# JuliaGraphics/Hikari.jl

Hardware: AMD Instinct MI355X
Metric: Mrays/s (higher is better)
Workload: dtype f32

## Files before the change

hikari.jl_amd/csrc/hk_kernels.hip:

```cpp
#include <hip/hip_runtime.h>
#include <type_traits>
#include <cstdlib>
#include <cstdio>

#include "hikari_mi355x.h"
#include "hk_device.h"
#include "hk_edit_host.h"
#include "hk_bvh_decide.h"

using namespace hkd;

namespace {

__device__ __forceinline__ int lane_id() { return (int)(threadIdx.x & 63); }

struct WaveQ {
    uint32_t* base;
    int count;
};
__device__ __forceinline__ int global_wave() {
    const int w = (int)(threadIdx.x >> 6), b = (int)blockIdx.x;
    if (blockDim.x == 1024 && (gridDim.x & 7) == 0) return ((((b >> 3) * 4 + (w >> 2)) * 8 + (b & 7)) << 2) + (w & 3);
    if (blockDim.x == 512 && (gridDim.x & 7) == 0) return ((((b >> 3) * 2 + (w >> 2)) * 8 + (b & 7)) << 2) + (w & 3);
    return b * (int)(blockDim.x >> 6) + w;
// ... 2197 lines not shown
                    if (descend) {
                        const int at = __popcll(dm & lt_mask);
                        pool[0][at] = e;
                        pool[1][at] = __float_as_uint(sp.x), pool[2][at] = __float_as_uint(sp.y), pool[3][at] = __float_as_uint(sp.z);
                        pool[4][at] = __float_as_uint(sn.x), pool[5][at] = __float_as_uint(sn.y), pool[6][at] = __float_as_uint(sn.z);
                        pool[7][at] = __float_as_uint(u_b);
                    }
                    pool_n = __popcll(dm);
                    __builtin_amdgcn_wave_barrier();
                }
            }
            const int avail = pool_n - pool_head;
            if (avail > 0) {
                const int rank = __popcll(free_m & lt_mask);
                if (!busy && rank < avail) {
                    const int at = pool_head + rank;
                    slot = pool[0][at];
                    p = mk3(__uint_as_float(pool[1][at]), __uint_as_float(pool[2][at]), __uint_as_float(pool[3][at]));
                    nn = mk3(__uint_as_float(pool[4][at]), __uint_as_float(pool[5][at]), __uint_as_float(pool[6][at]));
                    ub = __uint_as_float(pool[7][at]);
                    pmf = 1.0f - p_inf;
                    bits = root_bits, child = root_child;
                    lvl = 0;
                    busy = true;
                }
                const int free_n = __popcll(free_m);
                pool_head += free_n < avail ? free_n : avail;
            }
            if (__ballot(busy) == 0ull) {
                if (!more && pool_head == pool_n) break;
                continue;
            }
        }
        if (busy) {
            int res_light = -1;
            float res_pmf = 0.0f;
            if (lvl >= 64) {
                res_light = 0;
            } else {
                ++lvl;
                DLightNode n0, n1;
                if (NTOP > 0 && (int)child + 1 < n_top) {
                    n0 = lds_light_node<NTOP>(top, (int)child), n1 = lds_light_node<NTOP>(top, (int)child + 1);
                    asm volatile("" : "+v"(n0.bits));
                } else
                    n0 = load_light_node(sc.lnodes, (int)child), n1 = load_light_node(sc.lnodes, (int)child + 1);
                const float c0 = node_importance(n0, p, nn);
                const float c1 = node_importance(n1, p, nn);
                n_lnodes += 2;
                if (c0 == 0.0f && c1 == 0.0f) {
                    res_light = 0;
                } else {
                    const float p0 = c0 / (c0 + c1);
                    if (ub < p0) {
                        pmf *= p0;
                        ub = ub / p0;
                        bits = n0.bits, child = n0.child1_or_light;
                    } else {
                        pmf *= (1.0f - p0);
                        ub = (ub - p0) / (1.0f - p0);
                        bits = n1.bits, child = n1.child1_or_light;
                    }
                    if ((bits & 2u) && lvl < 64) {
                        res_light = (int)child;
                        res_pmf = pmf;
                    }
                }
            }
            if (res_light >= 0) {
                st.sel_light[slot] = make_uint2((uint32_t)res_light, __float_as_uint(res_pmf));
                busy = false;
            }
        }
    }
    stats += global_wave();
    wave_add(&stats->light_nodes, n_lnodes);
}

#ifndef HK_SHADE_WAVES_MATTE
#define HK_SHADE_WAVES_MATTE 4
#endif
#ifndef HK_SHADE_WAVES
#define HK_SHADE_WAVES 3
#endif
#ifndef HK_SHADE_WAVES_LEAN
#define HK_SHADE_WAVES_LEAN 5
#endif
#ifndef HK_SHADE_WAVES_LEAN_HASH
#define HK_SHADE_WAVES_LEAN_HASH 5
#endif
template <bool TWO_PLANES, bool SIMPLE, bool LEAN = false>
HKD void shade_emission(const DPathState& st, const DPathGen& g, bool ones, const DScene& sc, const DTables& T, uint32_t slot, unsigned& n_lnodes, int depth, size_t seg) {
    const float4 H = st.hit[slot];
    const float4 O = ld_ray_o(st, g, slot, depth, seg), D = g.ray_d[slot];
    const v3 ro = mk3(O.x, O.y, O.z), rd = mk3(D.x, D.y, D.z);
    const float t_hit = H.x;
    const int prim = __float_as_int(H.y);
    const DTriMeta meta = tri_meta(sc, prim);
    if (meta.arealight <= 0) return;
    const Surface sf = surface_at(sc, prim, H.z, H.w, ro, rd, t_hit);
    const v3 wo = -rd;
    uint2 pmeta;
    if constexpr (LEAN) {
        const uint32_t w = reinterpret_cast<const uint32_t*>(g.meta)[slot];
        pmeta = make_uint2((uint32_t)depth | (((w >> 30) & 1u) << 8), w & 0x3fffffffu);
    } else
        pmeta = ld_meta(st, g, slot, depth);
    const S4 lambda = ld_lambda(st, g, slot, pmeta.y);
    const DLight& light = sc.lights[meta.arealight - 1];
    S4 Le = arealight_Le<TWO_PLANES, SIMPLE>(sc, T, light, wo, sf.n, sf.uv, lambda);
    if (is_black(Le)) return;
    const S4 beta = ld_throughput(g.beta, slot, ones);
    const uint32_t fl = pmeta.x;
    const int pdepth = (int)(fl & 0xff);
    const bool specular_bounce = (fl >> 8) & 1u;
    S4 contribution = beta * Le;
    S4 fin;
    if constexpr (LEAN) {
        fin = contribution;
        if (!(pdepth == 0 || specular_bounce)) {
            const float r_l = ones ? 1.0f : D.w;
            float choice = bvh_pmf(sc, sf.pi, sf.n, (int)meta.arealight, n_lnodes);
            float ct = fabsf(dot(sf.n, normalize(rd)));
            float light_pdf = 0.0f;
            if (ct > 0.0f && sf.area > 0.0f) light_pdf = choice * ((t_hit * t_hit) / (ct * sf.area));
            const float a = 1.0f + r_l * light_pdf;
            const float den = (((a + a) + a) + a) / 4.0f;
            if (den > 1e-10f) fin = contribution / den;
        }
    } else {
        const S4 r_u = ld_ru(g, slot, ones, st.compact != 0), r_l = ld_rl(g, slot, ones, st.compact != 0);
        if (pdepth == 0 || specular_bounce)
            fin = contribution / average(r_u);
        else {
            float choice = bvh_pmf(sc, sf.pi, sf.n, (int)meta.arealight, n_lnodes);
            float ct = fabsf(dot(sf.n, normalize(rd)));
            float light_pdf = 0.0f;
            if (ct > 0.0f && sf.area > 0.0f) light_pdf = choice * ((t_hit * t_hit) / (ct * sf.area));
            S4 rl = r_l * light_pdf;
            float den = average(r_u + rl);
            fin = den > 1e-10f ? contribution / den : contribution / average(r_u);
        }
    }
    st4(&st.L[pmeta.y], ld4(&st.L[pmeta.y]) + fin);
}

template <int KIND>
struct ShadeWaves {
    static constexpr int value = (KIND == HK_MAT_COATED_DIFFUSE || KIND == HK_MAT_COATED_DIFFUSE_TRANSMISSION) ? 1 : (KIND == HK_MAT_MATTE ? HK_SHADE_WAVES_MATTE : HK_SHADE_WAVES);
};
#ifndef HK_SHADE_MIN_WAVES
#define HK_SHADE_MIN_WAVES 1
#endif
#define HK_SHADE_STASH 16
struct ShadeStage {
    uint32_t* entry;
    float4* hit;
    float4* ray_d;
    uint32_t* meta;
};
__device__ __forceinline__ void lds_fetch4(const uint32_t* src, uint32_t* lds_wave_base) {
    __builtin_amdgcn_global_load_lds((const __attribute__((address_space(1))) void*)src, (__attribute__((address_space(3))) void*)lds_wave_base, 4, 0, 0);
}
__device__ __forceinline__ void lds_fetch16(const float4* src, float4* lds_wave_base) {
    __builtin_amdgcn_global_load_lds((const __attribute__((address_space(1))) void*)src, (__attribute__((address_space(3))) void*)lds_wave_base, 16, 0, 0);
}
template <int KIND, bool SIMPLE, bool FT, bool PRE, bool LEAN = false>
__device__ __forceinline__ void shade_body(const DPathState& st, const DScene& sc, const DTables& T, const DFrame& fr, const DSobol& sob, int depth, int first_kind, DStats* stats, const SegTickets& src,
                                           uint32_t* __restrict__ elist,
                                           float* stash = nullptr,
                                           ShadeStage stage = ShadeStage{}) {
    static_assert(!LEAN || (KIND == HK_MAT_MATTE && HK_LAMBDA_BY_SLOT), "the lean body is Matte's");
    const int lane = lane_id();
    unsigned n_vertices = 0, n_lnodes = 0;
    unsigned nv_wave = 0;
    unsigned* const nl_stash = LEAN ? reinterpret_cast<unsigned*>(stash) + (HK_SHADE_STASH - 1) * 256 + threadIdx.x : nullptr;
    auto nl_flush = [&]() {
        if constexpr (LEAN) {
            if (n_lnodes) *nl_stash += n_lnodes;
            n_lnodes = 0;
        }
    };
    if constexpr (LEAN) *nl_stash = 0u;
    auto uni = [](int v) { return LEAN ? __builtin_amdgcn_readfirstlane(v) : v; };
    HK_FOR_EACH_SEGMENT_FROM(gw_v, st, src) {
    const int gw = uni(gw_v);
    const uint32_t* __restrict__ queue = st.mat_q + ((size_t)KIND * st.n_waves + gw) * st.wave_cap;
    const int n = uni(*count_ptr(st, depth, Q_MAT0 + KIND, gw));
    const DPathGen g = gen_at(st, depth), gn = st.gen[(depth + 1) & 1];
    const size_t seg = (size_t)gw * st.wave_cap;
    const bool ones = depth == 0 && fr.implicit_ones;
    WavePos q_shadow{0}, q_next{0};
    if (!first_kind) {
        q_shadow.count = uni(*count_ptr(st, depth, Q_SHADOW, gw));
        q_next.count = uni(*count_ptr(st, depth + 1, Q_RAY, gw));
    }
    int n_emit = 0;
    auto emit_pass = [&](int take) {
        __builtin_amdgcn_fence(__ATOMIC_SEQ_CST, "wavefront");
        if (lane < take) shade_emission<KIND == HK_MAT_MATTE, SIMPLE, LEAN>(st, g, ones, sc, T, elist[lane], n_lnodes, depth, seg);
        nl_flush();
        const int rest = n_emit - take;
        const uint32_t moved = lane < rest ? elist[64 + lane] : 0u;
        __builtin_amdgcn_fence(__ATOMIC_SEQ_CST, "wavefront");
        if (lane < rest) elist[lane] = moved;
        n_emit = rest;
    };
    const bool prescan = uni(st.shade_prescan) != 0;
    if (prescan) {
        for (int base = 0; base < n || n_emit > 0; base += 64) {
            if (base < n) {
                const int i = base + lane;
                const uint32_t cand = i < n ? queue[i] & ~HK_MATQ_EMISSIVE : 0u;
                const bool em = i < n && (st.mat_id[cand] & HK_MAT_EMISSIVE_BIT) != 0;
                const unsigned long long m = __ballot(em);
                if (em) elist[n_emit + __popcll(m & ((1ull << lane) - 1ull))] = cand;
                n_emit += __popcll(m);
                if (n_emit < 64 && base + 64 < n) continue;
            }
            emit_pass(n_emit < 64 ? n_emit : 64);
        }
    }
    const bool prefetch = LEAN && stage.entry != nullptr;
    const int wave0 = LEAN ? __builtin_amdgcn_readfirstlane((int)(threadIdx.x & ~63u)) : 0;
    if constexpr (LEAN) {
        if (prefetch && 64 + lane < n) lds_fetch4(&queue[64 + lane], stage.entry + 256 + wave0);
    }
    for (int base = 0; base < n; base += 64) {
        int i = base + lane;
        bool active = i < n;
        if constexpr (LEAN) {
            if (prefetch && i + 128 < n) lds_fetch4(&queue[i + 128], stage.entry + ((base >> 6) & 1) * 256 + wave0);
        }
        const bool staged = prefetch && base > 0;
        uint32_t slot = active ? queue[i] : 0u;
        {
            const bool em = !prescan && (slot & HK_MATQ_EMISSIVE) != 0u;
            slot &= ~HK_MATQ_EMISSIVE;
            const unsigned long long m = __ballot(em);
            if (m != 0ull) {
                if (em) elist[n_emit + __popcll(m & ((1ull << lane) - 1ull))] = slot;
                n_emit += __popcll(m);
                if (n_emit >= 64) emit_pass(64);
            }
        }
        bool push_shadow = false, push_ray = false;
        float4 H = make_float4(0, 0, 0, 0);
        Surface sf;
        v3 wo = mk3(0, 0, 1);
        DTriMeta meta{0u, 0u, 0u};
        S4 lambda = s4(0.0f), beta = s4(0.0f), r_u = s4(0.0f), kd_matte = s4(0.0f);
        uint32_t fl = 0, pslot = 0;
        int pdepth = 0, medium = -1;
        bool any_non_specular = false;
        SobolCtx sctx;
        using W = std::conditional_t<LEAN, float, S4>;
        auto stash_at = [&]() {
            int i = (int)threadIdx.x;
            asm volatile("" : "+v"(i));
            return stash + i;
        };
        const int base_dim = 6 + 7 * depth;
        float4 shO = make_float4(0, 0, 0, 0), shD = shO;
        S4 shLd = s4(0.0f);
        W shRu{}, shRl{};
        if constexpr (LEAN) nv_wave += (unsigned)(n - base < 64 ? n - base : 64);
        if (active) {
            if constexpr (!LEAN) ++n_vertices;
            float4 D;
            uint32_t meta_w = 0;
            if (LEAN && staged) {
                asm volatile("s_waitcnt vmcnt(0)" ::: "memory");
                const int t = (int)threadIdx.x;
                H = stage.hit[t], D = stage.ray_d[t], meta_w = stage.meta[t];
            } else {
                H = stream_ld(&st.hit[slot]);
                D = stream_ld(&g.ray_d[slot]);
                if constexpr (LEAN) meta_w = reinterpret_cast<const uint32_t*>(g.meta)[slot];
            }
            float4 O = ld_ray_o(st, g, slot, depth, seg);
            v3 ro = mk3(O.x, O.y, O.z), rd = mk3(D.x, D.y, D.z);
            float t_hit = H.x;
            int prim = __float_as_int(H.y);
            sf = surface_at(sc, prim, H.z, H.w, ro, rd, t_hit);
            wo = -rd;
            meta = tri_meta(sc, prim);
            if constexpr (LEAN) {
                pslot = meta_w & 0x3fffffffu;
                pdepth = depth;
                any_non_specular = (meta_w >> 31) != 0u;
            } else {
                const uint2 pmeta = ld_meta(st, g, slot, depth);
                fl = pmeta.x;
                pslot = pmeta.y;
                pdepth = (int)(fl & 0xff);
                any_non_specular = (fl >> 9) & 1u;
                medium = (int)(fl >> 16) - 1;
                r_u = ld_ru(g, slot, ones, st.compact != 0);
            }
            lambda = ld_lambda(st, g, slot, pslot);
            if (ones)
                beta = s4(1.0f);
            else {
                const float4 bv = stream_ld(&g.beta[slot]);
                beta = s4(bv.x, bv.y, bv.z, bv.w);
            }

            int pix, k;
            split_slot(fr, pslot, pix, k);
            sctx = sobol_ctx_slot(sob, T.sobol, fr.x0, fr.y0, fr.tiles_x, pix, k, fr.first_sample + k * fr.sample_stride);

            if (KIND == HK_MAT_MATTE) kd_matte = matte_kd<SIMPLE>(sc, T, sc.materials[st.mat_id[slot] & ~HK_MAT_EMISSIVE_BIT], TexCtx(sf.uv, meta.prim_index, H.z, H.w), lambda);
#ifdef HK_ABLATE
            {
                float sink = 0.0f;
                if (HK_ABLATE == 1) {
                    uint32_t ps2 = pslot;
                    int d2 = base_dim;
                    asm volatile("" : "+v"(ps2));
                    asm volatile("" : "+s"(d2));
                    int pix2, k2;
                    split_slot(fr, ps2, pix2, k2);
                    SobolCtx c2 = sobol_ctx_slot(sob, T.sobol, fr.x0, fr.y0, fr.tiles_x, pix2, k2, fr.first_sample + k2 * fr.sample_stride);
                    v2 a = sobol_2d(c2, d2 + 3), b = sobol_2d(c2, d2 + 6);
                    sink = sobol_1d(c2, d2 + 1) + a.x + a.y + b.x + b.y + sobol_1d(c2, d2 + 7);
                }
                if (HK_ABLATE == 2 && sc.n_lights > 0) {
                    float u2 = H.z, pmf2;
                    asm volatile("" : "+v"(u2));
                    unsigned dummy = 0;
                    sink = (float)bvh_sample_light(sc, sf.pi, sf.ns, u2, pmf2, dummy) + pmf2;
                }
                if (HK_ABLATE == 3 && sc.n_lights > 0) {
                    uint32_t li = pslot;
                    asm volatile("" : "+v"(li));
                    LightSample l2 = sample_light(sc, T, sc.lights[li % (uint32_t)sc.n_lights], sf.pi, lambda, mk2(H.z, H.w));
                    sink = l2.pdf + l2.Li.x + l2.Li.w + l2.wi.x + l2.p_light.z;
                }
                if (HK_ABLATE == 4) {
                    S4 l2 = lambda;
                    asm volatile("" : "+v"(l2.x), "+v"(l2.y), "+v"(l2.z), "+v"(l2.w));
                    S4 k2 = matte_kd(sc, T, sc.materials[st.mat_id[slot] & ~HK_MAT_EMISSIVE_BIT], TexCtx(sf.uv, meta.prim_index, H.z, H.w), l2);
                    sink = k2.x + k2.y + k2.z + k2.w;
                }
                if (HK_ABLATE == 5) {
                    float b2 = H.z;
                    asm volatile("" : "+v"(b2));
                    Surface s2 = surface_at(sc, prim, b2, H.w, ro, rd, t_hit);
                    sink = s2.pi.x + s2.n.y + s2.ns.z + s2.uv.x + s2.area;
                }
                if (HK_ABLATE == 6) {
                    v3 w2 = wo;
                    asm volatile("" : "+v"(w2.x), "+v"(w2.y), "+v"(w2.z));
                    float p2;
                    S4 f2 = eval_matte_kd(kd_matte, w2, sf.n, sf.ns, p2);
                    BSDFSample s2 = sample_matte_kd(sc, sc.materials[st.mat_id[slot] & ~HK_MAT_EMISSIVE_BIT], kd_matte, w2, sf.ns, TexCtx(sf.uv, meta.prim_index, H.z, H.w), mk2(H.z, H.w));
                    sink = f2.x + f2.w + p2 + s2.pdf + s2.wi.x + s2.f.y;
                }
                asm volatile("" : : "v"(sink));
            }
#endif

            if constexpr (LEAN) {
                float* sp = stash + threadIdx.x;
                sp[0 * 256] = sf.n.x, sp[1 * 256] = sf.n.y, sp[2 * 256] = sf.n.z;
                sp[3 * 256] = wo.x, sp[4 * 256] = wo.y, sp[5 * 256] = wo.z;
                sp[6 * 256] = kd_matte.x, sp[7 * 256] = kd_matte.y, sp[8 * 256] = kd_matte.z, sp[9 * 256] = kd_matte.w;
                sp[10 * 256] = beta.x, sp[11 * 256] = beta.y, sp[12 * 256] = beta.z, sp[13 * 256] = beta.w;
                sp[14 * 256] = __uint_as_float(meta_w);
                if (prefetch && i + 64 < n) {
                    asm volatile("s_waitcnt vmcnt(0)" ::: "memory");
                    const uint32_t ns = stage.entry[(((base >> 6) + 1) & 1) * 256 + (int)threadIdx.x] & ~HK_MATQ_EMISSIVE;
                    lds_fetch16(&st.hit[ns], stage.hit + wave0);
                    lds_fetch16(&g.ray_d[ns], stage.ray_d + wave0);
                    lds_fetch4(reinterpret_cast<const uint32_t*>(g.meta) + ns, stage.meta + wave0);
                }
            }
            if (sc.n_lights > 0) {
                const DMaterial& mat = sc.materials[st.mat_id[slot] & ~HK_MAT_EMISSIVE_BIT];
                float light_pmf;
                int light_idx;
                if constexpr (PRE) {
                    const uint2 pre = st.sel_light[slot];
                    light_idx = (int)pre.x;
                    light_pmf = __uint_as_float(pre.y);
                } else {
                    float light_select = sobol_1d<FT>(sctx, base_dim + 1);
                    light_idx = bvh_sample_light(sc, sf.pi, sf.ns, light_select, light_pmf, n_lnodes);
                }
                if (light_idx >= 1 && light_idx <= sc.n_lights && light_pmf > 0.0f) {
                    const DLight& sel = sc.lights[light_idx - 1];
                    v2 u_light = mk2(0.0f, 0.0f);
                    if (sel.kind >= HK_LIGHT_AMBIENT) u_light = sobol_2d<FT>(sctx, base_dim + 3);
                    LightSample ls = sample_light<KIND == HK_MAT_MATTE, SIMPLE>(sc, T, sel, sf.pi, lambda, u_light);
                    if (ls.pdf > 0.0f && !is_black(ls.Li)) {
                        float bsdf_pdf;
                        if constexpr (LEAN) {
                            const float* sp = stash_at();
                            wo = mk3(sp[3 * 256], sp[4 * 256], sp[5 * 256]);
                            kd_matte = s4(sp[6 * 256], sp[7 * 256], sp[8 * 256], sp[9 * 256]);
                            beta = s4(sp[10 * 256], sp[11 * 256], sp[12 * 256], sp[13 * 256]);
                        }
                        S4 f = KIND == HK_MAT_MATTE ? eval_matte_kd(kd_matte, wo, ls.wi, sf.ns, bsdf_pdf)
                                                    : eval_bsdf<KIND>(sc, T, mat, wo, ls.wi, sf.ns, TexCtx(sf.uv, meta.prim_index, H.z, H.w), lambda, bsdf_pdf);
                        if (!is_black(f)) {
                            float ct = fabsf(dot(ls.wi, sf.ns));
                            S4 Ld = beta * f * ls.Li * ct;
                            if (!is_black(Ld)) {
                                v3 off = 1e-4f * sf.ns;
                                v3 so = dot(ls.wi, sf.ns) > 0.0f ? sf.pi + off : sf.pi - off;
                                v3 tl = ls.p_light - so;
                                float tmax = sqrtf(dot(tl, tl)) - 1e-3f;
                                float nbp = ls.is_delta ? 0.0f : bsdf_pdf;
                                shO = make_float4(so.x, so.y, so.z, tmax);
                                shD = make_float4(ls.wi.x, ls.wi.y, ls.wi.z, __int_as_float(medium));
                                shLd = Ld;
                                if constexpr (LEAN) {
                                    shRu = nbp;
                                    shRl = ls.pdf * light_pmf;
                                } else {
                                    shRu = r_u * nbp;
                                    shRl = (r_u * ls.pdf) * light_pmf;
                                }
                                push_shadow = true;
                            }
                        }
                    }
                }
            }
        }
        nl_flush();
        {
            const size_t ps = seg + (size_t)wp_push(q_shadow, push_shadow);
            if constexpr (LEAN) {
                if (push_shadow) {
                    const float m = shRu + shRl;
                    shD.w = (((m + m) + m) + m) / 4.0f;
                    stream_st(&st.sh_o[ps], shO);
                    stream_st(&st.sh_d[ps], shD);
                    stream_st(&st.sh_Ld[ps], shLd);
                    stream_st(&st.sh_slot[ps], pslot);
                }
            } else if (push_shadow && st.sh_final) {
                const S4 mis = s4(shRu.x) * s4(1.0f) + s4(shRl.x) * s4(1.0f);
                shD.w = average(mis);
                stream_st(&st.sh_o[ps], shO);
                stream_st(&st.sh_d[ps], shD);
                stream_st(&st.sh_Ld[ps], shLd);
                stream_st(&st.sh_slot[ps], pslot);
            } else if (push_shadow) {
                stream_st(&st.sh_o[ps], shO);
                stream_st(&st.sh_d[ps], shD);
                stream_st(&st.sh_Ld[ps], shLd);
                if (st.compact) {
#if HK_NT
                    __builtin_nontemporal_store((hk_f2){shRu.x, shRl.x}, (hk_f2*)(reinterpret_cast<float2*>(st.sh_ru) + ps));
#else
                    reinterpret_cast<float2*>(st.sh_ru)[ps] = make_float2(shRu.x, shRl.x);
#endif
                } else
                    st_shadow_weights(st, ps, shRu, shRl);
                stream_st(&st.sh_slot[ps], pslot);
            }
        }
        float4 nO = make_float4(0, 0, 0, 0), nD = nO;
        S4 nb = s4(0.0f);
        W nrl{};
        uint32_t nflags = 0;
        if (active) {
            int new_depth = pdepth + 1;
            if (new_depth < fr.max_depth) {
                const DMaterial& mat = sc.materials[st.mat_id[slot] & ~HK_MAT_EMISSIVE_BIT];
                DMediumInterface mi{};
                if constexpr (LEAN) {
                    const float* sp = stash_at();
                    sf.n = mk3(sp[0 * 256], sp[1 * 256], sp[2 * 256]);
                    wo = mk3(sp[3 * 256], sp[4 * 256], sp[5 * 256]);
                    kd_matte = s4(sp[6 * 256], sp[7 * 256], sp[8 * 256], sp[9 * 256]);
                    beta = s4(sp[10 * 256], sp[11 * 256], sp[12 * 256], sp[13 * 256]);
                    const uint32_t meta_w = __float_as_uint(sp[14 * 256]);
                    pslot = meta_w & 0x3fffffffu;
                    any_non_specular = (meta_w >> 31) != 0u;
                    int pix, k;
                    split_slot(fr, pslot, pix, k);
                    sctx = sobol_ctx_slot(sob, T.sobol, fr.x0, fr.y0, fr.tiles_x, pix, k, fr.first_sample + k * fr.sample_stride);
                } else
                    mi = sc.mis[meta.mi];
                float uc = (KIND == HK_MAT_GLASS || KIND > HK_MAT_CONDUCTOR) && KIND != HK_MAT_FALLBACK ? sobol_1d<FT>(sctx, base_dim + 4) : 0.0f;
                v2 u = (KIND == HK_MAT_MIRROR || KIND == HK_MAT_GLASS || KIND == HK_MAT_THIN_DIELECTRIC) ? mk2(0.0f, 0.0f) : sobol_2d<FT>(sctx, base_dim + 6);
                bool regularize = fr.regularize && any_non_specular;
                BSDFSample s = KIND == HK_MAT_MATTE ? sample_matte_kd<SIMPLE>(sc, mat, kd_matte, wo, sf.ns, TexCtx(sf.uv, meta.prim_index, H.z, H.w), u)
                                                    : sample_bsdf<KIND>(sc, T, mat, wo, sf.ns, TexCtx(sf.uv, meta.prim_index, H.z, H.w), lambda, u, uc, regularize);
                if (s.pdf > 0.0f && !is_black(s.f)) {
                    float ct = fabsf(dot(s.wi, sf.ns));
                    nb = s.is_specular ? beta * s.f : beta * s.f * ct / s.pdf;
                    if constexpr (LEAN) nrl = s.is_specular ? 1.0f : 1.0f / s.pdf;
                    else nrl = s.is_specular ? r_u : r_u / s.pdf;
                    bool cont = true;
                    if (new_depth > 3) {
                        float rr = sobol_1d<FT>(sctx, base_dim + 7);
                        float q = maxf(0.05f, 1.0f - max_component(nb));
                        if (rr < q)
                            cont = false;
                        else
                            nb = nb * (1.0f / (1.0f - q));
                    }
                    if (cont) {
                        int new_medium = -1;
                        if constexpr (!LEAN) new_medium = (mi.inside != mi.outside) ? (dot(s.wi, sf.n) > 0.0f ? mi.outside : mi.inside) : medium;
                        v3 off = dot(s.wi, sf.n) > 0.0f ? sf.n : -sf.n;
                        v3 no = sf.pi + off * 0.0001f;
                        nO = make_float4(no.x, no.y, no.z, INF_F);
                        nD = make_float4(s.wi.x, s.wi.y, s.wi.z, 0.0f);
                        bool ans = any_non_specular || !s.is_specular;
                        nflags = (uint32_t)new_depth | ((s.is_specular ? 1u : 0u) << 8) | ((ans ? 1u : 0u) << 9) | ((uint32_t)(new_medium + 1) << 16);
                        push_ray = true;
                    }
                }
            }
        }
        {
            const size_t pn = seg + (size_t)wp_push(q_next, push_ray);
            if constexpr (LEAN) {
                if (push_ray) {
                    stream_st(&gn.ray_o[pn], nO);
                    nD.w = nrl;
                    stream_st(&gn.ray_d[pn], nD);
                    stream_st(&gn.beta[pn], nb);
                    stream_st(reinterpret_cast<uint32_t*>(gn.meta) + pn, pslot | (((nflags >> 8) & 1u) << 30) | (((nflags >> 9) & 1u) << 31));
                }
            } else if (push_ray) {
                stream_st(&gn.ray_o[pn], nO);
                if (st.compact) nD.w = nrl.x;
                stream_st(&gn.ray_d[pn], nD);
                stream_st(&gn.beta[pn], nb);
                st_ru_rl(gn, pn, r_u, nrl, st.compact != 0);
                st_lambda(gn, pn, lambda);
                st_meta(st, gn, pn, nflags, pslot);
            }
        }
    }
    if (n_emit > 0) emit_pass(n_emit);
    if (lane == 0) {
        *count_ptr(st, depth, Q_SHADOW, gw) = q_shadow.count;
        *count_ptr(st, depth + 1, Q_RAY, gw) = q_next.count;
    }
    }
    if constexpr (LEAN) {
        n_vertices = lane == 0 ? nv_wave : 0u;
        n_lnodes = *nl_stash;
    }
    stats += global_wave();
    wave_add(&stats->vertices, n_vertices);
    wave_add(&stats->light_nodes, n_lnodes);
}
template <int KIND, bool SIMPLE = false, bool FT = false, bool PRE = false, bool LEAN = false>
__global__ void __attribute__((amdgpu_flat_work_group_size(256, 256), amdgpu_waves_per_eu(LEAN ? (FT ? HK_SHADE_WAVES_LEAN : HK_SHADE_WAVES_LEAN_HASH) : ShadeWaves<KIND>::value))) k_shade(DPathState st, DScene sc, DTables T, DFrame fr, DSobol sob, int depth, int first_kind, DStats* stats) {
    __shared__ uint32_t emit_list[4 * 128];
    SegTickets src = seg_open(st, ticket_ptr(st, depth, TK_SHADE0 + KIND), st.dynamic_segments != 0, depth, Q_MAT0 + KIND);
    if constexpr (LEAN) {
        src.pos = __builtin_amdgcn_readfirstlane(src.pos), src.k0 = __builtin_amdgcn_readfirstlane(src.k0);
        __shared__ float stash[HK_SHADE_STASH * 256];
        __shared__ uint32_t stage_entry[2 * 256];
        __shared__ float4 stage_hit[256];
        __shared__ float4 stage_ray_d[256];
        __shared__ uint32_t stage_meta[256];
        ShadeStage stage{};
        if (st.shade_prefetch) stage.entry = stage_entry, stage.hit = stage_hit, stage.ray_d = stage_ray_d, stage.meta = stage_meta;
        shade_body<KIND, SIMPLE, FT, PRE, true>(st, sc, T, fr, sob, depth, first_kind, stats, src, emit_list + (threadIdx.x >> 6) * 128, stash, stage);
    } else
        shade_body<KIND, SIMPLE, FT, PRE>(st, sc, T, fr, sob, depth, first_kind, stats, src, emit_list + (threadIdx.x >> 6) * 128);
}

template <class W> HKD W wone();
template <> HKD float wone<float>() { return 1.0f; }
template <> HKD S4 wone<S4>() { return s4(1.0f); }
HKD S4 wide(S4 v) { return v; }
HKD S4 wide(float v) { return s4(v); }
HKD bool is_black(float v) { return v == 0.0f; }
template <bool COMPACT>
HKD void shadow_contribute(const DPathState& st, uint32_t rec, S4 T_ray, S4 tr_u, S4 tr_l) {
    if (is_black(T_ray)) return;
    S4 w_u, w_l;
    ld_shadow_weights<COMPACT>(st, rec, w_u, w_l);
    S4 mis = w_u * tr_u + w_l * tr_l;
    float den = average(mis);
    if (den > 1e-10f) {
        S4 fin = ld4(&st.sh_Ld[rec]) * T_ray / den;
        if (!is_black(fin)) {
            const uint32_t pslot = st.sh_slot[rec];
            st4(&st.L[pslot], ld4(&st.L[pslot]) + fin);
        }
    }
}

HKD void shadow_contribute_final(const DPathState& st, uint32_t rec, float den) {
    if (den > 1e-10f) {
        const S4 fin = ld4(&st.sh_Ld[rec]) * s4(1.0f) / den;
        if (!is_black(fin)) {
            const uint32_t pslot = st.sh_slot[rec];
            st4(&st.L[pslot], ld4(&st.L[pslot]) + fin);
        }
    }
}
HKD void shadow_contribute_rt(const DPathState& st, uint32_t rec, S4 T_ray, S4 tr_u, S4 tr_l) {
    if (st.compact)
        shadow_contribute<true>(st, rec, T_ray, tr_u, tr_l);
    else
        shadow_contribute<false>(st, rec, T_ray, tr_u, tr_l);
}

template <bool COUNT, int NC, bool QN = false>
__device__ __forceinline__ void shadow_body(const DPathState& st, const DScene& sc, int depth, DStats* stats, SegStream stream, int* __restrict__ stack, const NodeCache& cache) {
    const int lane = lane_id();
    const unsigned long long lt_mask = (1ull << lane) - 1ull;
    const int DONE = (int)0x80000000;
    unsigned n_nodes = 0, n_tris = 0, n_casts = 0, n_hits = 0;
    HK_DBG_DECL
    uint32_t seg = 0;
    int n = 0, cursor = 0;
    bool more = true;
    bool have = false;
    uint32_t slot = 0;
    float rec_den = 0.0f;
    LaneRay r;
    r.cur = r.pend = DONE;
    for (;;) {
        const unsigned long long run_m = __ballot(have && r.cur != DONE);
        if (run_m == 0ull || (64 - __popcll(run_m) >= HK_TRACE_MIN_IDLE && (cursor < n || more))) {
            if (have && r.cur == DONE) {
                if (r.best.prim < 0) {
                    if (st.sh_final)
                        shadow_contribute_final(st, slot, rec_den);
                    else
                        shadow_contribute<true>(st, slot, s4(1.0f), s4(1.0f), s4(1.0f));
                } else
                    ++n_hits;
                have = false;
            }
            while (more && cursor >= n) {
                const int gw = stream_next(stream, st.n_waves);
                if (gw >= st.n_waves) {
                    more = false;
                    break;
                }
                seg = (uint32_t)gw * (uint32_t)st.wave_cap;
                n = *count_ptr(st, depth, Q_SHADOW, gw);
                cursor = 0;
            }
            const unsigned long long want = __ballot(!have);
            const int avail = n - cursor;
            const int rank = __popcll(want & lt_mask);
            if (!have && rank < avail) {
                slot = seg + (uint32_t)(cursor + rank);
                float4 O = stream_ld(&st.sh_o[slot]), D = stream_ld(&st.sh_d[slot]);
                rec_den = D.w;
                if (O.w >= 1e-6f) {
                    ++n_casts;
                    lane_ray_start<QN>(r, sc, mk3(O.x, O.y, O.z), mk3(D.x, D.y, D.z), O.w);
                    have = true;
                }
            }
            const int want_n = __popcll(want);
            cursor += want_n < avail ? want_n : (avail > 0 ? avail : 0);
            if (__ballot(have) == 0ull) {
                if (cursor >= n && !more) break;
                continue;
            }
        }
#ifdef HK_DEBUG_UTIL
        HK_DBG(5, have && r.cur != DONE);
        lane_ray_round<true, COUNT, NC, HK_POSTPONE_ANYHIT != 0, false, QN>(r, have && r.cur != DONE, sc, stack, lane, n_nodes, n_tris, cache, cursor < n || more, dbg_ + 6);
#else
        lane_ray_round<true, COUNT, NC, HK_POSTPONE_ANYHIT != 0, false, QN>(r, have && r.cur != DONE, sc, stack, lane, n_nodes, n_tris, cache, cursor < n || more);
#endif
    }
    stats += global_wave();
    HK_DBG_FLUSH(stats);
    wave_add(&stats->rays_shadow, n_casts);
    wave_add(&stats->hits, n_hits);
    if (COUNT) {
        wave_add(&stats->sh_nodes, n_nodes);
        wave_add(&stats->sh_tris, n_tris);
    }
}
template <bool COUNT, int STACK, int BLOCK = HK_TRACE_BLOCK, int NC = 0, bool QN = false>
__global__ void __launch_bounds__(BLOCK) k_shadow(DPathState st, DScene sc, int depth, DStats* stats) {
    __shared__ int lds_stack[(BLOCK / 64) * STACK * 64];
    __shared__ float4 lds_box[NC > 0 ? 3 * NC : 1];
    __shared__ int2 lds_child[NC > 0 ? NC : 1];
    int* stack = lds_stack + (threadIdx.x >> 6) * (STACK * 64);
    const NodeCache cache = node_cache_fill<NC, BLOCK, QN>(sc, lds_box, lds_child);
    shadow_body<COUNT, NC, QN>(st, sc, depth, stats, stream_open(st, ticket_ptr(st, depth, TK_SHADOW), false, depth, Q_SHADOW), stack, cache);
}

template <int NC>
__device__ __forceinline__ void trace_shadow_body(const DPathState& st, const DScene& sc, int depth, DStats* stats, int gw, int* __restrict__ stack, const NodeCache& cache) {
    const int lane = lane_id();
    const unsigned long long lt_mask = (1ull << lane) - 1ull;
    const int DONE = (int)0x80000000;
    unsigned n_nodes = 0, n_tris = 0, n_casts = 0, n_hits = 0, n_sh_casts = 0;
    const int dt = depth + 1;
    const DPathGen g = gen_at(st, dt);
    const uint32_t seg = (uint32_t)gw * (uint32_t)st.wave_cap;
    const int n_ray = *count_ptr(st, dt, Q_RAY, gw), n_sh = *count_ptr(st, depth, Q_SHADOW, gw);
    WaveQ q_escaped = wq_open(st.escaped_q, st, gw);
    int kind_count[HK_MAX_KINDS];
#pragma unroll
    for (int k = 0; k < HK_MAX_KINDS; ++k) kind_count[k] = 0;
    int cur_ray = 0, cur_sh = 0;
    int state = LR_EMPTY;
    uint32_t slot = 0;
    float rec_den = 0.0f;
    LaneRay r;
    r.cur = r.pend = DONE;
    r.any = false;
    for (;;) {
        const unsigned long long run_m = __ballot(state == LR_ACTIVE && r.cur != DONE);
        if (run_m == 0ull || (64 - __popcll(run_m) >= HK_TRACE_MIN_IDLE && (cur_ray < n_ray || cur_sh < n_sh))) {
            int kind = -1;
            uint32_t eflag = 0u;
// ... 2050 lines not shown
```

hikari.jl_amd/csrc/hk_render.cpp:

```cpp
#include "hk_host.h"

namespace {
float gaussian_1d(float x, float sigma) { return std::exp(-(x * x) / (2.0f * (sigma * sigma))); }
float mitchell_1d(float x, float B, float C) {
    x = std::fabs(x);
    if (x <= 1.0f) return ((12.0f - 9.0f * B - 6.0f * C) * (x * x * x) + (-18.0f + 12.0f * B + 6.0f * C) * (x * x) + (6.0f - 2.0f * B)) / 6.0f;
    if (x <= 2.0f) return ((-B - 6.0f * C) * (x * x * x) + (6.0f * B + 30.0f * C) * (x * x) + (-12.0f * B - 48.0f * C) * x + (8.0f * B + 24.0f * C)) / 6.0f;
    return 0.0f;
}
float sinc1(float x) {
    x = std::fabs(x);
    if (x < 1e-5f) return 1.0f;
    x *= 3.14159265358979323846f;
    return std::sin(x) / x;
}
float wsinc(float x, float r, float tau) {
    x = std::fabs(x);
    if (x > r) return 0.0f;
    return sinc1(x) * sinc1(x / tau);
}
float filter_eval(const hk_integrator_params& p, float ex, float ey, float x, float y) {
    float rx = p.filter_radius[0], ry = p.filter_radius[1];
    switch (p.filter_type) {
        case HK_FILTER_BOX: return (std::fabs(x) <= rx && std::fabs(y) <= ry) ? 1.0f : 0.0f;
// ... 61 lines not shown
        HIP_TRY(I->f_mcdf.upload(mcdf.data(), mcdf.size() * 4));
        HIP_TRY(I->f_mfunc.upload(mfunc.data(), mfunc.size() * 4));
        HIP_TRY(I->f_ccdf.upload(ccdf.data(), ccdf.size() * 4));
        f.nx = nx;
        f.ny = ny;
        f.func = I->f_func.as<float>();
        f.marginal_cdf = I->f_mcdf.as<float>();
        f.marginal_func = I->f_mfunc.as<float>();
        f.conditional_cdf = I->f_ccdf.as<float>();
        f.dmin_x = dmin_x;
        f.dmin_y = dmin_y;
        f.dmax_x = dmax_x;
        f.dmax_y = dmax_y;
        f.func_integral = func_integral;
    }
    *out = I;
    return HK_OK;
}
extern "C" int32_t hk_integrator_destroy(hk_integrator* I) {
    int status = HK_OK;
    if (I) {
        (void)hipSetDevice(I->ctx->device);
        status = join_lanes(I->ctx);
        if (hipStreamSynchronize(I->ctx->stream) != hipSuccess && status == HK_OK) status = fail(HK_ERR_DEVICE, "hk_integrator_destroy: the context's stream reports an error");
        quiesce(I->ctx);
        delete I;
    }
    return status;
}

namespace {
template <class T>
hipError_t alloc_arr(hk_integrator* I, T*& dst, size_t n) {
    if (I->slab_mode != 0) {
        const size_t bytes = (n * sizeof(T) + ((size_t)2 << 20) - 1) & ~(((size_t)2 << 20) - 1);
        dst = I->slab_mode == 2 ? reinterpret_cast<T*>(static_cast<char*>(I->slab_base) + I->slab_off) : nullptr;
        I->slab_off += bytes;
        return hipSuccess;
    }
    I->bufs.emplace_back(new DevBuf());
    DevBuf* b = I->bufs.back().get();
    hipError_t e = b->alloc(n * sizeof(T));
    dst = b->as<T>();
    return e;
}
struct PassTraits {
    bool media, open_scene, small_scene, grey_compact;
    bool fusable;
    bool lean;
};
PassTraits pass_traits(const hk_scene* sc, const hk_ctx* c, int n_samples, bool piped) {
    PassTraits t;
    t.media = sc->d.n_media > 0;
    t.open_scene = sc->d.has_escape_lights != 0;
    t.small_scene = sc->d.bvh_depth <= 16;
    t.grey_compact = sc->d.n_media > 0 && hk::grey_compact_ok(sc->d);
    t.fusable = !piped && !c->time_kernels && !c->count_nodes && n_samples < 16 && hk::small_pass_fusable(sc->d, sc->kinds_mask);
    t.lean = hk::lean_scene(sc->d);
    return t;
}
int layout_state(hk_integrator* I, bool media, bool want_split, bool want_cam) {
    DPathState& s = I->st;
    const size_t P = (size_t)s.capacity, Q = (size_t)s.n_waves * s.wave_cap;
    const int n_cu = I->ctx->n_cu, W = s.n_waves;
    for (int gidx = 0; gidx < 2; ++gidx) {
        DPathGen& g = s.gen[gidx];
        HIP_TRY(alloc_arr(I, g.ray_o, Q));
        HIP_TRY(alloc_arr(I, g.ray_d, Q));
        HIP_TRY(alloc_arr(I, g.beta, Q));
        HIP_TRY(alloc_arr(I, g.r_u, Q));
        HIP_TRY(alloc_arr(I, g.r_l, Q));
#if HK_LAMBDA_BY_SLOT
        g.lambda = nullptr;
#else
        HIP_TRY(alloc_arr(I, g.lambda, Q));
#endif
        HIP_TRY(alloc_arr(I, g.meta, Q));
    }
    HIP_TRY(alloc_arr(I, s.hit, Q));
    HIP_TRY(alloc_arr(I, s.mat_id, Q));
    s.sel_light = nullptr;
    if (!media) HIP_TRY(alloc_arr(I, s.sel_light, Q));
    HIP_TRY(alloc_arr(I, s.lambda_s, P));
    s.pdf = nullptr;
    HIP_TRY(alloc_arr(I, s.L, P));
    HIP_TRY(alloc_arr(I, s.filter_w, P));
    HIP_TRY(alloc_arr(I, s.sh_o, Q));
    HIP_TRY(alloc_arr(I, s.sh_d, Q));
    HIP_TRY(alloc_arr(I, s.sh_Ld, Q));
    HIP_TRY(alloc_arr(I, s.sh_ru, Q));
    HIP_TRY(alloc_arr(I, s.sh_rl, Q));
    HIP_TRY(alloc_arr(I, s.sh_slot, Q));
    s.sh_T = nullptr, s.sh_aux = nullptr, s.sh_it = nullptr, s.wq_a = nullptr, s.wq_b = nullptr, s.wq_ctl = nullptr;
    if (want_split) {
        HIP_TRY(alloc_arr(I, s.sh_T, Q));
        HIP_TRY(alloc_arr(I, s.sh_aux, Q));
        HIP_TRY(alloc_arr(I, s.sh_it, 4 * Q));
        const size_t wq_n = (Q / 193 + 1) * 256 + (size_t)256 * 32 * (size_t)n_cu;
        HIP_TRY(alloc_arr(I, s.wq_a, wq_n));
        HIP_TRY(alloc_arr(I, s.wq_b, wq_n));
        HIP_TRY(alloc_arr(I, s.wq_ctl, (size_t)(I->p.max_depth + 2) * 11 * 4));
    }
    HIP_TRY(alloc_arr(I, s.escaped_q, Q));
    HIP_TRY(alloc_arr(I, s.medium_q, Q));
    HIP_TRY(alloc_arr(I, s.scatter_q, Q));
    s.ticket_rows = I->p.max_depth + 2;
    HIP_TRY(alloc_arr(I, s.tickets, (size_t)s.ticket_rows * HK_TICKET_COLS * HK_TICKET_WAYS * HK_TICKET_STRIDE));
    HIP_TRY(alloc_arr(I, s.initial_medium, 1));
    if (I->slab_mode != 1) HIP_TRY(hipMemset(s.initial_medium, 0xff, sizeof(int)));
    HIP_TRY(alloc_arr(I, s.mat_q, Q * HK_MAX_KINDS));
    size_t nc = (size_t)(I->p.max_depth + 2) * Q_COUNT * W;
    HIP_TRY(alloc_arr(I, s.counters, nc));
    if (I->slab_mode != 1) HIP_TRY(hipMemset(s.counters, 0, nc * sizeof(int)));
    HIP_TRY(alloc_arr(I, s.seg_list, nc));
    HIP_TRY(alloc_arr(I, s.seg_list_n, (size_t)(I->p.max_depth + 2) * Q_COUNT));
    I->cam_gen = DPathGen{};
    I->cam_unfit = false;
    if (want_cam) {
        DPathGen g{};
        uint32_t* meta32 = nullptr;
        const size_t n_bufs = I->bufs.size();
        if (alloc_arr(I, g.ray_o, Q) == hipSuccess && alloc_arr(I, g.ray_d, Q) == hipSuccess && alloc_arr(I, meta32, Q) == hipSuccess) {
            g.meta = reinterpret_cast<uint2*>(meta32);
            I->cam_gen = g;
        } else {
            (void)hipGetLastError();
            I->bufs.resize(n_bufs);
            I->cam_unfit = true;
        }
    }
    return HK_OK;
}
int ensure_state(hk_integrator* I, int capacity, const PassTraits& t, hipStream_t users) {
    const bool media = t.media, open_scene = t.open_scene, small_scene = t.small_scene, grey_compact = t.grey_compact, fusable = t.fusable, lean = t.lean;
    const int n_cu = I->ctx->n_cu;
    long mid_paths = 48L << 20;
    if (const char* e = hk::knob("HK_MID_PASS_PATHS_M")) mid_paths = std::atol(e) >= 0 ? std::atol(e) << 20 : mid_paths;
    const bool mid = !media && !open_scene && small_scene && (long)capacity <= mid_paths;
    I->mid_pass = mid;
    const long cap_per_cu = media ? 96 : ((open_scene || mid) ? 48 : 192);
    long W_want = ((long)(capacity + 63) / 64) / 16;
    if (W_want < 4L * n_cu) W_want = 4L * n_cu;
    if (W_want > cap_per_cu * n_cu) W_want = cap_per_cu * n_cu;
    I->ctx->waves_per_cu = hk::knob_int_in("HK_WAVES_PER_CU", 1, INT_MAX, 0);
    if (I->ctx->waves_per_cu > 0) W_want = (long)I->ctx->waves_per_cu * n_cu;
    W_want = (W_want + 3) / 4 * 4;
    I->st.dynamic_segments = (media || (!open_scene && !mid)) ? 1 : 0;
    I->st.dynamic_segments = hk::knob_int("HK_DYNAMIC_SEGMENTS", I->st.dynamic_segments) ? 1 : 0;
    I->st.compact = media ? (grey_compact ? 1 : 0) : 1;
    I->st.sh_final = (lean && hk::knob_on("HK_SHADOW_FINAL")) ? 1 : 0;
    I->st.meta32 = (lean && hk::knob_on("HK_LEAN_RECORDS")) ? 1 : 0;
    I->st.const_origin = 0;
    I->st.shade_prescan = hk::knob_int("HK_SHADE_PRESCAN", 0) != 0 ? 1 : 0;
    I->st.shade_prefetch = hk::knob_on("HK_SHADE_PREFETCH") ? 1 : 0;
    I->st.ticket_share = hk::knob_int("HK_TICKET_SHARE", 1) ? 1 : 0;
    {
        const bool small_on = hk::knob_on("HK_SMALL_PASS");
        const bool small = W_want <= 4L * n_cu && small_on && hk::knob("HK_DYNAMIC_SEGMENTS") == nullptr;
        I->st.small_pass = small ? 1 : 0;
        if (mid && I->st.dynamic_segments == 0 && small_on && !hk::knob_int("HK_MID_LISTS", 0))
            I->st.small_pass = 1;
        if (small) {
            I->st.dynamic_segments = 0;
            const int w = hk::knob_int_in("HK_SMALL_PASS_WAVES", 1, INT_MAX, 0);
            long per_cu = w > 0 ? w : (users ? (media ? 4 : 8) : (((open_scene && !media) || fusable) ? 8 : 16));
            const long chunks = ((long)capacity + 63) / 64;
            while (per_cu > 4 && per_cu * n_cu > chunks) per_cu /= 2;
            if (I->ctx->waves_per_cu <= 0) W_want = (per_cu * n_cu + 3) / 4 * 4;
        }
    }
    const bool want_split = media && hk::walk_split_mode();
    const bool want_cam = !media && !users && hk::knob_on("HK_VIEW_CACHE");
    if (I->st_capacity >= capacity && I->st_depth >= I->p.max_depth && I->st.n_waves == (int)W_want && I->st_media == (media ? 1 : 0) && (!want_split || I->st.wq_a != nullptr) &&
        (!want_cam || I->cam_gen.ray_d != nullptr || I->cam_unfit))
        return HK_OK;
    I->view_key.clear();
    if (users) HIP_TRY(hipStreamSynchronize(users));
    if (!I->bufs.empty()) quiesce(I->ctx);
    I->bufs.clear();
    DPathState& s = I->st;
    const int W = (int)W_want;
    const int chunks = (capacity + 63) / 64;
    s.capacity = capacity;
    s.n_waves = W;
    s.wave_cap = ((chunks + W - 1) / W) * 64;
    if ((size_t)W * (size_t)s.wave_cap > 0x7fffffffu) return fail(HK_ERR_INVALID, "pass too large");
    if (hk::knob_on("HK_STATE_SLAB")) {
        bool cam = want_cam;
        for (;;) {
            I->slab_mode = 1, I->slab_off = 0;
            if (int e = layout_state(I, media, want_split, cam)) {
                I->slab_mode = 0;
                return e;
            }
            size_t free_b = 0, total_b = 0;
            const bool known = hipMemGetInfo(&free_b, &total_b) == hipSuccess;
            if (!known) (void)hipGetLastError();
            hipError_t he = hipErrorOutOfMemory;
            if (!(cam && known && I->slab_off > free_b + g_slabs.total(I->ctx->device))) {
                I->bufs.emplace_back(new DevBuf());
                he = I->bufs.back()->alloc_slab(I->ctx->device, I->slab_off);
            }
            if (he == hipSuccess) break;
            (void)hipGetLastError();
            I->bufs.clear();
            if (!cam) {
                I->slab_mode = 0;
                return fail(HK_ERR_DEVICE, "path-state slab allocation failed");
            }
            cam = false;
        }
        I->slab_base = I->bufs.back()->p;
        I->slab_mode = 2, I->slab_off = 0;
        const int e = layout_state(I, media, want_split, cam);
        I->slab_mode = 0;
        if (e) return e;
        I->cam_unfit = want_cam && !cam;
    } else if (int e = layout_state(I, media, want_split, want_cam))
        return e;
    I->st_capacity = capacity;
    I->st_depth = I->p.max_depth;
    I->st_media = media ? 1 : 0;
    if (hk::knob("HK_DEBUG_ALLOC"))
        std::fprintf(stderr, "HK_DEBUG_ALLOC capacity %d Q %zu: ray_o %p ray_d %p beta %p hit %p sh_o %p L %p medium_q %p mat_q %p counters %p\n", capacity, (size_t)W * s.wave_cap, (void*)s.gen[0].ray_o,
                     (void*)s.gen[0].ray_d, (void*)s.gen[0].beta, (void*)s.hit, (void*)s.sh_o, (void*)s.L, (void*)s.medium_q, (void*)s.mat_q, (void*)s.counters);
    return HK_OK;
}
}
int ceil_log2(long v) {
    int l = 0;
    while ((1L << l) < v) ++l;
    return l;
}
DSobol make_sobol(const hk_integrator_params& p, int w, int h) {
    DSobol s;
    int spp = p.samples_per_pixel > 4096 ? p.samples_per_pixel : 4096;
    s.log2_spp = ceil_log2(spp < 1 ? 1 : spp);
    int res_log2 = ceil_log2(w > h ? w : h);
    s.n_base4_digits = res_log2 + (s.log2_spp + 1) / 2;
    s.seed = p.sampler_seed;
    s.width = w;
    s.hi_table = nullptr;
    s.hi_rows = s.hi_stride = 0;
    s.lo_table = nullptr;
    s.lo_rows = s.lo_count = s.lo_offset = 0;
    return s;
}

namespace {
int choose_samples_per_pass(hk_ctx* c, const hk_integrator* I, const DFrame& fr, int n_samples, int& S_out) {
    int S = I->p.samples_per_pass;
    if (S <= 0) {
        long max_paths = 192L << 20;
        if (const char* e = hk::knob("HK_MAX_PATHS_M")) max_paths = std::atol(e) > 0 ? std::atol(e) << 20 : max_paths;
        S = (int)(max_paths / fr.n_pixels_padded);
        if (S < 1) S = 1;
        if (S > 256) S = 256;
        size_t free_b = 0, total_b = 0;
        if (hipMemGetInfo(&free_b, &total_b) == hipSuccess) {
            free_b += g_slabs.total(c->device);
            while (S > 1 && (size_t)S * fr.n_pixels_padded * 440 > free_b / 2) S /= 2;
        }
    }
    if (S > n_samples) S = n_samples;
    if ((long)S * fr.n_pixels_padded > 0x3fffffffL) return fail(HK_ERR_INVALID, "pass too large");
    S_out = S;
    return HK_OK;
}
int pick_lane(hk_ctx* c, hk_integrator* I, const DFrame& fr, int S, int n_samples, int& lane_idx) {
    lane_idx = -1;
    int n_lanes = 1;
    long max_paths = 8L << 20;
    n_lanes = hk::knob_int_in("HK_PIPELINE", 1, 16, n_lanes);
    if (const char* e = hk::knob("HK_PIPELINE_MAX_PATHS_M")) max_paths = std::atol(e) > 0 ? std::atol(e) << 20 : max_paths;
    {
        const long by_memory = (8L << 30) / (440L * (long)S * fr.n_pixels_padded);
        if (n_lanes > by_memory) n_lanes = by_memory < 1 ? 1 : (int)by_memory;
    }
    const bool small_call = n_samples <= S && (long)S * fr.n_pixels_padded <= max_paths;
    int after = 4;
    after = hk::knob_int_in("HK_PIPELINE_AFTER", 0, INT_MAX, after);
    c->small_streak = small_call ? c->small_streak + 1 : 0;
    const bool lanes_started = c->ev_main != nullptr;
    if (n_lanes > 1 && !c->time_kernels && small_call && (lanes_started || c->small_streak > after)) {
        if ((int)I->lane_sets.size() < (int)hk_ctx::MAX_LANES) I->lane_sets.resize(hk_ctx::MAX_LANES);
        lane_idx = c->next_lane % n_lanes;
        c->next_lane = (lane_idx + 1) % n_lanes;
        hk_ctx::Lane& L = c->lanes[lane_idx];
        if (!L.stream) HIP_TRY(hipStreamCreateWithFlags(&L.stream, hipStreamNonBlocking));
        if (!L.done) {
            HIP_TRY(hipEventCreateWithFlags(&L.done, hipEventDisableTiming));
            std::vector<DStats> zero((size_t)c->stat_rows);
            std::memset(zero.data(), 0, zero.size() * sizeof(DStats));
            HIP_TRY(L.stats.upload(zero.data(), zero.size() * sizeof(DStats)));
        }
        if (!c->ev_main) {
            HIP_TRY(hipEventCreateWithFlags(&c->ev_main, hipEventDisableTiming));
            HIP_TRY(hipEventCreateWithFlags(&c->ev_film, hipEventDisableTiming));
        }
    } else {
        if (int e = join_lanes(c)) return e;
    }
    return HK_OK;
}
int ensure_sobol_tables(hk_ctx* c, hk_integrator* I, const DFrame& fr, DSobol& sob, int first_sample_idx, int n_samples, int sample_stride) {
    const int x0 = fr.x0, y0 = fr.y0;
    const int rows = 4 + 5 * (I->p.max_depth + 1);
// ... 370 lines not shown
```

Baseline: 10990.

## Stage queue entries, material ids and beta through LDS in lean matte shading

Extends the lean Matte shading prefetch so that material ids, the next queue entries and per-path beta are loaded asynchronously into LDS via global_load_lds, rather than read from global memory inside the loop. Beta and material now live in dedicated LDS arrays instead of the per-thread register stash, so the stash shrinks from 16 to 12 slots. The prefetch default is changed to the new full mode (level 2). In exchange it adds more LDS per block and extra s_waitcnt points, which may reduce occupancy or serialize loads.

Measured after the change: 11070, median of 6. No clear change (+0.7%).

```diff
diff --git a/hikari.jl_amd/csrc/hk_kernels.hip b/hikari.jl_amd/csrc/hk_kernels.hip
--- a/hikari.jl_amd/csrc/hk_kernels.hip
+++ b/hikari.jl_amd/csrc/hk_kernels.hip
@@ -2373,12 +2373,15 @@
 #ifndef HK_SHADE_MIN_WAVES
 #define HK_SHADE_MIN_WAVES 1
 #endif
-#define HK_SHADE_STASH 16
+#define HK_SHADE_STASH 12
 struct ShadeStage {
     uint32_t* entry;
     float4* hit;
     float4* ray_d;
     uint32_t* meta;
+    uint32_t* mat;
+    float4* beta;
+    bool full;
 };
 __device__ __forceinline__ void lds_fetch4(const uint32_t* src, uint32_t* lds_wave_base) {
     __builtin_amdgcn_global_load_lds((const __attribute__((address_space(1))) void*)src, (__attribute__((address_space(3))) void*)lds_wave_base, 4, 0, 0);
@@ -2443,6 +2446,7 @@
         }
     }
     const bool prefetch = LEAN && stage.entry != nullptr;
+    const bool full = LEAN && prefetch && stage.full;
     const int wave0 = LEAN ? __builtin_amdgcn_readfirstlane((int)(threadIdx.x & ~63u)) : 0;
     if constexpr (LEAN) {
         if (prefetch && 64 + lane < n) lds_fetch4(&queue[64 + lane], stage.entry + 256 + wave0);
@@ -2450,11 +2454,20 @@
     for (int base = 0; base < n; base += 64) {
         int i = base + lane;
         bool active = i < n;
-        if constexpr (LEAN) {
-            if (prefetch && i + 128 < n) lds_fetch4(&queue[i + 128], stage.entry + ((base >> 6) & 1) * 256 + wave0);
-        }
+        const int half = LEAN ? ((base >> 6) & 1) * 256 : 0;
         const bool staged = prefetch && base > 0;
-        uint32_t slot = active ? queue[i] : 0u;
+        uint32_t slot;
+        if (LEAN && staged && full) {
+            asm volatile("s_waitcnt vmcnt(0)" ::: "memory");
+            slot = 0u;
+            if (active) slot = stage.entry[half + (int)threadIdx.x];
+            asm volatile("" : "+v"(slot));
+        } else {
+            if constexpr (LEAN) {
+                if (prefetch && i + 128 < n) lds_fetch4(&queue[i + 128], stage.entry + half + wave0);
+            }
+            slot = active ? queue[i] : 0u;
+        }
         {
             const bool em = !prescan && (slot & HK_MATQ_EMISSIVE) != 0u;
             slot &= ~HK_MATQ_EMISSIVE;
@@ -2481,6 +2494,20 @@
             asm volatile("" : "+v"(i));
             return stash + i;
         };
+        auto beta_landed = [&]() {
+            if (full && !ones) asm volatile("s_waitcnt vmcnt(0)" ::: "memory");
+        };
+        auto beta_back = [&]() {
+            int i = (int)threadIdx.x;
+            asm volatile("" : "+v"(i));
+            const float4 b = stage.beta[i];
+            return s4(b.x, b.y, b.z, b.w);
+        };
+        auto mat_back = [&]() {
+            int i = half + (int)threadIdx.x;
+            asm volatile("" : "+v"(i));
+            return stage.mat[i];
+        };
         const int base_dim = 6 + 7 * depth;
         float4 shO = make_float4(0, 0, 0, 0), shD = shO;
         S4 shLd = s4(0.0f);
@@ -2490,14 +2517,24 @@
             if constexpr (!LEAN) ++n_vertices;
             float4 D;
             uint32_t meta_w = 0;
+            uint32_t mat_w = 0;
             if (LEAN && staged) {
-                asm volatile("s_waitcnt vmcnt(0)" ::: "memory");
+                if (!full) asm volatile("s_waitcnt vmcnt(0)" ::: "memory");
                 const int t = (int)threadIdx.x;
                 H = stage.hit[t], D = stage.ray_d[t], meta_w = stage.meta[t];
+                if (full) mat_w = stage.mat[half + t];
             } else {
                 H = stream_ld(&st.hit[slot]);
                 D = stream_ld(&g.ray_d[slot]);
                 if constexpr (LEAN) meta_w = reinterpret_cast<const uint32_t*>(g.meta)[slot];
+            }
+            if (!(LEAN && staged && full)) mat_w = st.mat_id[slot];
+            if constexpr (LEAN) {
+                if (full) {
+                    asm volatile("s_waitcnt lgkmcnt(0)" : "+v"(slot) : : "memory");
+                    if (staged && i + 128 < n) lds_fetch4(&queue[i + 128], stage.entry + half + wave0);
+                    if (!ones) lds_fetch16(&g.beta[slot], stage.beta + wave0);
+                }
             }
             float4 O = ld_ray_o(st, g, slot, depth, seg);
             v3 ro = mk3(O.x, O.y, O.z), rd = mk3(D.x, D.y, D.z);
@@ -2522,7 +2559,7 @@
             lambda = ld_lambda(st, g, slot, pslot);
             if (ones)
                 beta = s4(1.0f);
-            else {
+            else if (!(LEAN && full)) {
                 const float4 bv = stream_ld(&g.beta[slot]);
                 beta = s4(bv.x, bv.y, bv.z, bv.w);
             }
@@ -2531,7 +2568,7 @@
             split_slot(fr, pslot, pix, k);
             sctx = sobol_ctx_slot(sob, T.sobol, fr.x0, fr.y0, fr.tiles_x, pix, k, fr.first_sample + k * fr.sample_stride);
 
-            if (KIND == HK_MAT_MATTE) kd_matte = matte_kd<SIMPLE>(sc, T, sc.materials[st.mat_id[slot] & ~HK_MAT_EMISSIVE_BIT], TexCtx(sf.uv, meta.prim_index, H.z, H.w), lambda);
+            if (KIND == HK_MAT_MATTE) kd_matte = matte_kd<SIMPLE>(sc, T, sc.materials[mat_w & ~HK_MAT_EMISSIVE_BIT], TexCtx(sf.uv, meta.prim_index, H.z, H.w), lambda);
 #ifdef HK_ABLATE
             {
                 float sink = 0.0f;
@@ -2587,18 +2624,20 @@
                 sp[0 * 256] = sf.n.x, sp[1 * 256] = sf.n.y, sp[2 * 256] = sf.n.z;
                 sp[3 * 256] = wo.x, sp[4 * 256] = wo.y, sp[5 * 256] = wo.z;
                 sp[6 * 256] = kd_matte.x, sp[7 * 256] = kd_matte.y, sp[8 * 256] = kd_matte.z, sp[9 * 256] = kd_matte.w;
-                sp[10 * 256] = beta.x, sp[11 * 256] = beta.y, sp[12 * 256] = beta.z, sp[13 * 256] = beta.w;
-                sp[14 * 256] = __uint_as_float(meta_w);
+                sp[10 * 256] = __uint_as_float(meta_w);
+                if (ones || !full) stage.beta[threadIdx.x] = make_float4(beta.x, beta.y, beta.z, beta.w);
+                if (!(staged && full)) stage.mat[half + (int)threadIdx.x] = mat_w;
                 if (prefetch && i + 64 < n) {
                     asm volatile("s_waitcnt vmcnt(0)" ::: "memory");
-                    const uint32_t ns = stage.entry[(((base >> 6) + 1) & 1) * 256 + (int)threadIdx.x] & ~HK_MATQ_EMISSIVE;
+                    const uint32_t ns = stage.entry[(half ^ 256) + (int)threadIdx.x] & ~HK_MATQ_EMISSIVE;
                     lds_fetch16(&st.hit[ns], stage.hit + wave0);
                     lds_fetch16(&g.ray_d[ns], stage.ray_d + wave0);
                     lds_fetch4(reinterpret_cast<const uint32_t*>(g.meta) + ns, stage.meta + wave0);
+                    if (full) lds_fetch4(reinterpret_cast<const uint32_t*>(st.mat_id) + ns, stage.mat + (half ^ 256) + wave0);
                 }
             }
             if (sc.n_lights > 0) {
-                const DMaterial& mat = sc.materials[st.mat_id[slot] & ~HK_MAT_EMISSIVE_BIT];
+                const DMaterial& mat = sc.materials[LEAN ? 0u : st.mat_id[slot] & ~HK_MAT_EMISSIVE_BIT];
                 float light_pmf;
                 int light_idx;
                 if constexpr (PRE) {
@@ -2620,7 +2659,8 @@
                             const float* sp = stash_at();
                             wo = mk3(sp[3 * 256], sp[4 * 256], sp[5 * 256]);
                             kd_matte = s4(sp[6 * 256], sp[7 * 256], sp[8 * 256], sp[9 * 256]);
-                            beta = s4(sp[10 * 256], sp[11 * 256], sp[12 * 256], sp[13 * 256]);
+                            beta_landed();
+                            beta = beta_back();
                         }
                         S4 f = KIND == HK_MAT_MATTE ? eval_matte_kd(kd_matte, wo, ls.wi, sf.ns, bsdf_pdf)
                                                     : eval_bsdf<KIND>(sc, T, mat, wo, ls.wi, sf.ns, TexCtx(sf.uv, meta.prim_index, H.z, H.w), lambda, bsdf_pdf);
@@ -2651,6 +2691,7 @@
             }
         }
         nl_flush();
+        if constexpr (LEAN) beta_landed();
         {
             const size_t ps = seg + (size_t)wp_push(q_shadow, push_shadow);
             if constexpr (LEAN) {
@@ -2691,15 +2732,15 @@
         if (active) {
             int new_depth = pdepth + 1;
             if (new_depth < fr.max_depth) {
-                const DMaterial& mat = sc.materials[st.mat_id[slot] & ~HK_MAT_EMISSIVE_BIT];
+                const DMaterial& mat = sc.materials[(LEAN ? mat_back() : st.mat_id[slot]) & ~HK_MAT_EMISSIVE_BIT];
                 DMediumInterface mi{};
                 if constexpr (LEAN) {
                     const float* sp = stash_at();
                     sf.n = mk3(sp[0 * 256], sp[1 * 256], sp[2 * 256]);
                     wo = mk3(sp[3 * 256], sp[4 * 256], sp[5 * 256]);
                     kd_matte = s4(sp[6 * 256], sp[7 * 256], sp[8 * 256], sp[9 * 256]);
-                    beta = s4(sp[10 * 256], sp[11 * 256], sp[12 * 256], sp[13 * 256]);
-                    const uint32_t meta_w = __float_as_uint(sp[14 * 256]);
+                    beta = beta_back();
+                    const uint32_t meta_w = __float_as_uint(sp[10 * 256]);
                     pslot = meta_w & 0x3fffffffu;
                     any_non_specular = (meta_w >> 31) != 0u;
                     int pix, k;
@@ -2786,8 +2827,12 @@
         __shared__ float4 stage_hit[256];
         __shared__ float4 stage_ray_d[256];
         __shared__ uint32_t stage_meta[256];
+        __shared__ uint32_t stage_mat[2 * 256];
+        __shared__ float4 stage_beta[256];
         ShadeStage stage{};
+        stage.mat = stage_mat, stage.beta = stage_beta;
         if (st.shade_prefetch) stage.entry = stage_entry, stage.hit = stage_hit, stage.ray_d = stage_ray_d, stage.meta = stage_meta;
+        stage.full = st.shade_prefetch >= 2;
         shade_body<KIND, SIMPLE, FT, PRE, true>(st, sc, T, fr, sob, depth, first_kind, stats, src, emit_list + (threadIdx.x >> 6) * 128, stash, stage);
     } else
         shade_body<KIND, SIMPLE, FT, PRE>(st, sc, T, fr, sob, depth, first_kind, stats, src, emit_list + (threadIdx.x >> 6) * 128);
diff --git a/hikari.jl_amd/csrc/hk_render.cpp b/hikari.jl_amd/csrc/hk_render.cpp
--- a/hikari.jl_amd/csrc/hk_render.cpp
+++ b/hikari.jl_amd/csrc/hk_render.cpp
@@ -237,7 +237,7 @@
     I->st.meta32 = (lean && hk::knob_on("HK_LEAN_RECORDS")) ? 1 : 0;
     I->st.const_origin = 0;
     I->st.shade_prescan = hk::knob_int("HK_SHADE_PRESCAN", 0) != 0 ? 1 : 0;
-    I->st.shade_prefetch = hk::knob_on("HK_SHADE_PREFETCH") ? 1 : 0;
+    I->st.shade_prefetch = hk::knob_int_in("HK_SHADE_PREFETCH", 0, 2, 2);
     I->st.ticket_share = hk::knob_int("HK_TICKET_SHARE", 1) ? 1 : 0;
     {
         const bool small_on = hk::knob_on("HK_SMALL_PASS");
```
